# bhargav0410/gpu-accel-ofdm-ls-mrc

Measured on AMD Instinct MI355X. Metric: OFDM symbols/s (LS+MRC) at 1024 subcarriers x 64 ant; achieved HBM GB/s vs peak, higher is better.
Workload: dtype f32; 1 GPU; OFDM uplink LS+MRC, time-domain IQ in HBM, 1250 frames x 101 symbols (1 pilot + 100 data) x 64 antennas x 1024 subcarriers per GPU; domain=time, R=64, C=1024, S=101, prefix=0, frames_per_gpu=1250, data_symbols_per_gpu=125000, global_data_symbols=125000, flow=one-launch, parallelism=frame-sharded x1, no collective

## Files before the change

### gpu-accel-ofdm-ls-mrc_amd/csrc/frame_td.hip

```cpp
#include "launch.hpp"
#include "wave_fft1024.hpp"
#include "diag.hpp"

OFDM_DIAG_TU(td1024)


namespace ofdm {
namespace td1024 {

constexpr int LS_WAVES = 4;

template <int NW, class IQ>
__global__ void __launch_bounds__(64 * NW) k_ls_td1024(const IQ *__restrict__ iq, int S, int R,
                                                       int prefix, const float2 *__restrict__ X,
                                                       float2 *__restrict__ Hc, float *__restrict__ P,
                                                       int partial, float scale) {
    extern __shared__ __attribute__((aligned(16))) float2 lds[];
    float2 *tw = lds;
    const int w = threadIdx.x >> 6;
    const int t = threadIdx.x & 63;
    float2 *T = lds + TWBUF + w * TBUF;
    fill_twiddles(tw);
    __syncthreads();

    const long long f = blockIdx.x;
    const int Cp = C + prefix;
    const IQ *pilot = iq + f * (long long)S * R * Cp + prefix;
    float4 *Hf = reinterpret_cast<float4 *>(Hc + f * (long long)R * C);
    const int b0 = lane_bin0(t);
    float2 xp[16];
#pragma unroll
    for (int k = 0; k < 16; ++k) {
        const int b = b0 + 16 * k;
        xp[k] = b > 0 ? X[b - 1] : float2{1.f, 0.f};
    }
    float p[16];
#pragma unroll
    for (int k = 0; k < 16; ++k) p[k] = 0.f;
    for (int r = w; r < R; r += NW) {
        float2 a[16], x[16];
        if constexpr (is_sc16<IQ>) {
            unsigned raw[16];
            row_load(pilot + (long long)r * Cp, t, raw);
            widen_row(raw, a);
        } else {
            row_load(pilot + (long long)r * Cp, t, a);
        }
        row_fft(a, t, T, tw, x);
#pragma unroll
        for (int k = 0; k < 16; ++k) {
            float2 h = ls_conj(x[k], xp[k]);
            if constexpr (is_sc16<IQ>) h = float2{h.x * scale, h.y * scale};
            if (b0 + 16 * k == 0) h = float2{0.f, 0.f};
            x[k] = h;
            p[k] = p[k] + (h.x * h.x) + (h.y * h.y);
        }
        hc_store(Hf + (long long)r * (C / 2), t, x);
    }
    __syncthreads();
    float *pp = reinterpret_cast<float *>(lds + TWBUF);
    static_assert(NW * C * sizeof(float) <= NW * TBUF * sizeof(float2), "partials fit the transpose images");
#pragma unroll
    for (int k = 0; k < 16; ++k) pp[w * C + b0 + 16 * k] = p[k];
    __syncthreads();
    float *Pf = P + f * C;
    const int nw = R < NW ? R : NW;
    for (int b = threadIdx.x; b < C; b += blockDim.x) {
        float sum = pp[b];
        for (int i = 1; i < nw; ++i) sum = sum + pp[i * C + b];
        Pf[b] = b == 0 ? (partial ? 0.f : 1.f) : sum;
    }
}


__device__ __forceinline__ void fft_a(float2 (&a)[16], int t, float2 *T, const float2 *tw1) {
    hlds::row_fft_a<0, false, true>(a, t, T, tw1);
}
__device__ __forceinline__ void fft_b(int t, float2 *T, const float2 *tw2, float2 (&x)[16]) {
    hlds::row_fft_b<0, false, true>(t, T, tw2, x);
}
__device__ __forceinline__ void mac(float2 &acc, float2 x, float vx, float vy) {
    acc.x = __builtin_fmaf(-x.y, vy, __builtin_fmaf(x.x, vx, acc.x));
    acc.y = __builtin_fmaf(x.y, vx, __builtin_fmaf(x.x, vy, acc.y));
}


typedef int v4i_t __attribute__((ext_vector_type(4)));
template <bool PREF, class IQ>
__device__ __forceinline__ void hlds_row_pf(const IQ *next, __amdgpu_buffer_rsrc_t hc, int hoff, int t,
                                            row_reg_t<IQ> (&a)[16],
                                            float2 *T, const float2 *tw1, const float2 *tw2,
                                            const float4 *lo, const float4 *hi, float4 *mine,
                                            float2 (&acc)[16]) {
    using namespace hlds;
    float2 x[16];
    if constexpr (is_sc16<IQ>) {
        float2 af[16];
        widen_row(a, af);
        fft_a(af, t, T, tw1);
    } else {
        fft_a(a, t, T, tw1);
    }
    const float4 hreg = __builtin_bit_cast(float4, (v4i_t)__builtin_amdgcn_raw_buffer_load_b128(hc, t * 16, hoff, 0));
    __builtin_amdgcn_sched_barrier(0);
    if (PREF) row_load<true>(next, t, a);
    fft_b(t, T, tw2, x);
    if constexpr (is_sc16<IQ>) __builtin_amdgcn_sched_barrier(0);
    lds_barrier();
    *mine = hreg;
    lds_barrier();
#pragma unroll
    for (int i = 0; i < 8; ++i) {
        const float4 v = i < 4 ? lo[i * 64] : hi[(i - 4) * TS];
        mac(acc[2 * i], x[2 * i], v.x, v.y);
        mac(acc[2 * i + 1], x[2 * i + 1], v.z, v.w);
    }
}

template <bool R0, class IQ>
__device__ __forceinline__ void row0(const IQ *sym, int t, const float2 *T, row_reg_t<IQ> (&a)[16]) {
    if constexpr (R0) {
        static_assert(!is_sc16<IQ>, "sc16 rows are only 4-byte aligned: no 16-B row-0 DMA");
        asm volatile("s_waitcnt vmcnt(0)" ::: "memory");
#pragma unroll
        for (int m = 0; m < 16; ++m) a[m] = T[t + 64 * m];
    } else {
        row_load<true>(sym, t, a);
    }
}
__device__ __forceinline__ void row0_dma(const float2 *sym, int t, float2 *T) {
    const char *src = reinterpret_cast<const char *>(sym) + t * 16;
    const unsigned dst = lds_addr(T);
#pragma unroll
    for (int j = 0; j < 8; ++j) dma16(src + j * 1024, dst + j * 1024);
}

template <bool SHARED, bool R0 = false, class IQ>
__device__ __forceinline__ void hlds_rows(const IQ *sym, int Cp, int R, const float4 *Hf, int t,
                                          float2 *T, const float2 *tw1, const float2 *tw2,
                                          float2 *T0, float4 *hfree, float2 (&acc)[16]) {
    using namespace hlds;
#pragma unroll
    for (int k = 0; k < 16; ++k) acc[k] = float2{0.f, 0.f};
    if constexpr (SHARED) {
        row_reg_t<IQ> a[16];
        const int tl = lane_here();
        row0<R0>(sym, tl, T, a);
        const float4 *lo = hfree + tl;
        const float4 *hi = hslot(T0, hfree, 256 + tl);
        float4 *mine = hslot(T0, hfree, threadIdx.x);
        const __amdgpu_buffer_rsrc_t hc =
            __builtin_amdgcn_make_buffer_rsrc(const_cast<float4 *>(Hf), (short)0, R * (C * 8), 0x00020000);
        const int hw = __builtin_amdgcn_readfirstlane(threadIdx.x >> 6) * 1024;
        for (int r = 0; r + 1 < R; ++r)
            hlds_row_pf<true>(sym + (long long)(r + 1) * Cp, hc, r * (C * 8) + hw, lane_here(), a, T, tw1, tw2, lo,
                              hi, mine, acc);
        hlds_row_pf<false>(sym, hc, (R - 1) * (C * 8) + hw, lane_here(), a, T, tw1, tw2, lo, hi, mine, acc);
    } else {
        for (int r = 0; r < R; ++r) {
            float2 a[16], x[16], h[16];
            if constexpr (is_sc16<IQ>) {
                unsigned raw[16];
                if (r == 0)
                    row0<R0>(sym, t, T, raw);
                else
                    row_load<true>(sym + (long long)r * Cp, t, raw);
                widen_row(raw, a);
            } else if (r == 0) {
                row0<R0>(sym, t, T, a);
            } else {
                row_load<true>(sym + (long long)r * Cp, t, a);
            }
            fft_a(a, t, T, tw1);
            fft_b(t, T, tw2, x);
            __builtin_amdgcn_sched_barrier(0);
            hc_load(Hf + (long long)r * (C / 2), t, h);
#pragma unroll
            for (int k = 0; k < 16; ++k) mac(acc[k], x[k], h[k].x, h[k].y);
        }
    }
}

template <bool SCALED = false>
__device__ __forceinline__ void hlds_epilogue(const float2 (&acc)[16], const float *P, long long f, long long q,
                                              int t, float2 *T, float2 *__restrict__ out, int mode,
                                              float scale = 1.f) {
    const int b0 = lane_bin0(t);
    float2 *o = out + q * K;
    const float *Pf = P + f * C + b0;
    float pv[16];
    if ((mode & 1) == 0) {
#pragma unroll
        for (int k = 0; k < 16; ++k) pv[k] = Pf[16 * k];
    }
#pragma unroll
    for (int k = 0; k < 16; ++k) {
        const int b = b0 + 16 * k;
        float2 v = acc[k];
        int j = b - 1;
        if ((mode & 1) == 0) {
            float rp = __builtin_amdgcn_rcpf(pv[k]);
            if constexpr (SCALED) rp = rp * scale;
            v = float2{acc[k].x * rp, acc[k].y * rp};
            j = out_pos(b > 0 ? b - 1 : 0, K);
        } else if constexpr (SCALED) {
            v = float2{acc[k].x * scale, acc[k].y * scale};
        }
        if (b > 0) T[(j >> 6) * hlds::TP + (j & 63)] = v;
    }
    wave_lds_sync();
#pragma unroll
    for (int m = 0; m < 16; ++m) {
        const int j = t + 64 * m;
        if (j < K) {
            const float2 v = T[m * hlds::TP + t];
            __builtin_nontemporal_store(__builtin_bit_cast(unsigned long long, v),
                                        reinterpret_cast<unsigned long long *>(o + j));
        }
    }
}

template <bool R0, class IQ>
__global__ void __attribute__((amdgpu_flat_work_group_size(512, 512), amdgpu_waves_per_eu(4, 4)))
k_mrc_td1024_hlds(const IQ *__restrict__ iq, int S, int R, int prefix, const float2 *__restrict__ Hc,
                  const float *__restrict__ P, float2 *__restrict__ out, long long nq, long long nblocks,
                  long long per_xcd, int mode, float scale) {
    using namespace hlds;
    constexpr int HW = WAVES;
    extern __shared__ __attribute__((aligned(16))) float2 lds[];
    float2 *tw1 = lds, *tw2 = lds + TW1S;
    const int w = __builtin_amdgcn_readfirstlane(threadIdx.x >> 6), t = threadIdx.x & 63;
    float2 *T = lds + TW1S + TW2S + w * TS;
    float2 *T0 = lds + TW1S + TW2S;
    float4 *hfree = reinterpret_cast<float4 *>(T0 + HW * TS);
    const long long pb = blockIdx.x;
    const long long lb = (pb & 7) * per_xcd + (pb >> 3);
    if (lb >= nblocks) return;

    const int nsym = S - 1;
    const long long qw = lb * HW + w;
    const bool store = qw < nq;
    const long long q = store ? qw : nq - 1;
    const long long f = uniform64(q / nsym);
    const long long f0 = (lb * HW) / nsym;
    const long long fl = ((lb * HW + HW - 1 < nq ? lb * HW + HW - 1 : nq - 1)) / nsym;
    const int s = 1 + (int)(q % nsym);
    const int Cp = C + prefix;
    const IQ *sym = iq + (f * S + s) * (long long)R * Cp + prefix;
    if constexpr (R0) row0_dma(sym, t, T);
    fill(tw1, tw2);
    __syncthreads();

    float2 acc[16];
    if (f0 == fl)
        hlds_rows<true, R0>(sym, Cp, R, reinterpret_cast<const float4 *>(Hc + f0 * (long long)R * C), t, T,
                                 tw1, tw2, T0, hfree, acc);
    else
        hlds_rows<false, R0>(sym, Cp, R, reinterpret_cast<const float4 *>(Hc + f * (long long)R * C), t, T,
                                tw1, tw2, T0, hfree, acc);
    if (!store) return;
    if constexpr (is_sc16<IQ>)
        hlds_epilogue<true>(acc, P, f, q, lane_here(), T, out, mode, scale);
    else
        hlds_epilogue(acc, P, f, q, lane_here(), T, out, mode);
}


__device__ __forceinline__ void hlds_ls_frame(const float2 *__restrict__ iq, int S, int R, int prefix,
                                              const float2 *__restrict__ X, float2 *Hc, float *P, long long f,
                                              int w, int t, float2 *T, float2 *T0, const float2 *tw1,
                                              const float2 *tw2, unsigned long long *mx = nullptr) {
    using namespace hlds;
    (void)mx;
    const int Cp = C + prefix;
    const float2 *pilot = iq + f * (long long)S * R * Cp + prefix;
    float4 *Hf = reinterpret_cast<float4 *>(Hc + f * (long long)R * C);
    const int b0 = lane_bin0(t);
    float2 xp[16];
#pragma unroll
    for (int k = 0; k < 16; ++k) {
        const int b = b0 + 16 * k;
        xp[k] = b > 0 ? X[b - 1] : float2{1.f, 0.f};
    }
    float p[16];
#pragma unroll
    for (int k = 0; k < 16; ++k) p[k] = 0.f;
    for (int r = w; r < R; r += WAVES) {
        float2 a[16], x[16];
        const int tl = lane_here();
        row_load<true>(pilot + (long long)r * Cp, tl, a);
        fft_a(a, tl, T, tw1);
        fft_b(tl, T, tw2, x);
#pragma unroll
        for (int k = 0; k < 16; ++k) {
            float2 h = ls_conj(x[k], xp[k]);
            if (b0 + 16 * k == 0) h = float2{0.f, 0.f};
            x[k] = h;
            p[k] = p[k] + (h.x * h.x) + (h.y * h.y);
        }
#pragma unroll
        for (int i = 0; i < 8; ++i) store16_wt(Hf, R * C * 8, (r * (C / 2) + i * 64 + tl) * 16, x[2 * i], x[2 * i + 1]);
        if (r == w) {
            OFDM_DIAG_MARKP(mx, 1)
        }
    }
    OFDM_DIAG_MARKP(mx, 2)
    __syncthreads();
    float *pp = reinterpret_cast<float *>(T0);
#pragma unroll
    for (int k = 0; k < 16; ++k) pp[w * C + b0 + 16 * k] = p[k];
    __syncthreads();
    float *Pf = P + f * C;
    const int nw = R < WAVES ? R : WAVES;
    for (int b = threadIdx.x; b < C; b += blockDim.x) {
        float sum = pp[b];
        for (int i = 1; i < nw; ++i) sum = sum + pp[i * C + b];
        const float v = b == 0 ? 1.f : sum;
        store4_wt(Pf + b, v);
    }
    OFDM_DIAG_MARKP(mx, 3)
    __syncthreads();
}

__device__ __forceinline__ void split_unit(const float2 *__restrict__ iq, int S, int R, int prefix, const float2 *Hc,
                                           const float *P, float2 *__restrict__ out, long long nq, long long q0, int w,
                                           int t, float2 *T, float2 *T0, const float2 *tw1, const float2 *tw2) {
    const int nsym = S - 1, Cp = C + prefix, hh = w >> 2, R0 = (R + 1) >> 1;
    const long long qw = q0 + (w & 3);
    const bool store = qw < nq;
    const long long q = store ? qw : nq - 1;
    const long long f = q / nsym;
    const int s = 1 + (int)(q % nsym);
    const float2 *sym = iq + (f * S + s) * (long long)R * Cp + prefix;
    const float4 *Hf = reinterpret_cast<const float4 *>(Hc + f * (long long)R * C);
    float2 acc[16];
#pragma unroll
    for (int k = 0; k < 16; ++k) acc[k] = float2{0.f, 0.f};
    const int r1 = hh ? R : R0;
    for (int r = hh ? R0 : 0; r < r1; ++r) {
        float2 a[16], x[16], h[16];
        row_load<true>(sym + (long long)r * Cp, t, a);
        fft_a(a, t, T, tw1);
        fft_b(t, T, tw2, x);
        __builtin_amdgcn_sched_barrier(0);
        hc_load(Hf + (long long)r * (C / 2), t, h);
#pragma unroll
        for (int k = 0; k < 16; ++k) mac(acc[k], x[k], h[k].x, h[k].y);
    }
    if (hh) {
#pragma unroll
        for (int k = 0; k < 16; ++k) T[k * hlds::TP + t] = acc[k];
    }
    __syncthreads();
    if (hh) return;
    const float2 *Tp = T0 + (w + 4) * hlds::TS;
#pragma unroll
    for (int k = 0; k < 16; ++k) {
        const float2 v = Tp[k * hlds::TP + t];
        acc[k] = float2{acc[k].x + v.x, acc[k].y + v.y};
    }
    if (store) hlds_epilogue(acc, P, f, q, t, T, out, 0);
}

__global__ void __attribute__((amdgpu_flat_work_group_size(512, 512), amdgpu_waves_per_eu(4, 4)))
k_demod_td1024(const float2 *__restrict__ iq, int S, int R, int prefix, const float2 *__restrict__ X, float2 *Hc,
               float *P, float2 *__restrict__ out, long long nq, long long nblocks, Tickets tk, long long k0, long long split, unsigned long long *flags, unsigned long long epoch,
               int nls, long long nframes, long long spin_ticks) {
    using namespace hlds;
    constexpr int HW = WAVES;
    extern __shared__ __attribute__((aligned(16))) float2 lds[];
    float2 *tw1 = lds, *tw2 = lds + TW1S;
    const int w = __builtin_amdgcn_readfirstlane(threadIdx.x >> 6), t = threadIdx.x & 63;
    float2 *T = lds + TW1S + TW2S + w * TS;
    float2 *T0 = lds + TW1S + TW2S;
    float4 *hfree = reinterpret_cast<float4 *>(T0 + HW * TS);
    OFDM_DIAG_BEGIN()

    const bool estimator = (int)blockIdx.x < nls;
    auto first_frame = [&](long long lb) { return (lb * HW) / (S - 1); };
    auto last_frame = [&](long long lb) { return ((lb * HW + HW - 1 < nq ? lb * HW + HW - 1 : nq - 1)) / (S - 1); };
    const int nsym = S - 1, Cp = C + prefix;
    auto sym_of = [&](long long lb) {
        const long long qw = lb * HW + w, q = qw < nq ? qw : nq - 1;
        return iq + ((q / nsym) * S + 1 + q % nsym) * (long long)R * Cp + prefix;
    };
    long long e0 = 1, e1 = 0, lb = 0;
    int um = 0;
    if (estimator) {
        e0 = e1 = blockIdx.x;
        if (e0 >= nframes) return;
        __builtin_amdgcn_s_setprio(3);
        fill(tw1, tw2);
        __syncthreads();
        OFDM_DIAG_MARKN(0)
    } else {
        FillRegs fr;
        fill_load(fr);
        lb = wg_take_unit(tk, nblocks, k0, (long long)blockIdx.x - nls, split,
                          reinterpret_cast<long long *>(hfree + 255));
        if (lb < 0) return;
        OFDM_DIAG_MARKN(0)
        um = (int)(lb & 3);
        lb >>= 2;
        fill_store(tw1, tw2, fr);
        const long long f0 = first_frame(lb), fl = last_frame(lb);
        if (!um) row0_dma(sym_of(lb), t, T);
        bool seen_before = false;
        if (threadIdx.x == 0)
            seen_before = __hip_atomic_load((gu64 *)(flags + f0), __ATOMIC_RELAXED, __HIP_MEMORY_SCOPE_AGENT) == epoch &&
                          __hip_atomic_load((gu64 *)(flags + fl), __ATOMIC_RELAXED, __HIP_MEMORY_SCOPE_AGENT) == epoch;
        OFDM_DIAG_MARKN(1)
        if (!consume_flags(flags, f0, fl, epoch, spin_ticks, reinterpret_cast<int *>(hfree), seen_before)) {
            asm volatile("s_waitcnt vmcnt(0)" ::: "memory");
            __syncthreads();
            e0 = f0;
            e1 = fl;
        }
    }
    for (long long ff = e0; ff <= e1; ++ff)
        hlds_ls_frame(iq, S, R, prefix, X, Hc, P, ff, w, t, T, T0, tw1, tw2, OFDM_DIAG_ARG);
    if (estimator) {
        OFDM_DIAG_MARK()
        publish_flag(flags + e0, epoch, w == 0 && lane_here() == 0);
        OFDM_DIAG_END_SLOT(td1024, epoch);
        return;
    }
    if (e0 <= e1) {
        acquire_all();
        if (!um) row0_dma(sym_of(lb), t, T);
    }
    OFDM_DIAG_MARK()

    if (um) {
        split_unit(iq, S, R, prefix, Hc, P, out, nq, lb * HW + 4 * (um - 1), w, t, T, T0, tw1, tw2);
        OFDM_DIAG_END_SLOT(td1024, epoch);
        return;
    }
    const long long qw = lb * HW + w;
    const bool store = qw < nq;
    const long long q = store ? qw : nq - 1;
    const long long f = q / nsym;
    const long long f0 = first_frame(lb), fl = last_frame(lb);
    const float2 *sym = sym_of(lb);
    float2 acc[16];
    if (f0 == fl)
        hlds_rows<true, true>(sym, Cp, R, reinterpret_cast<const float4 *>(Hc + f0 * (long long)R * C), t, T,
                              tw1, tw2, T0, hfree, acc);
    else
        hlds_rows<false, true>(sym, Cp, R, reinterpret_cast<const float4 *>(Hc + f * (long long)R * C), t, T,
                               tw1, tw2, T0, hfree, acc);
    OFDM_DIAG_MARKN(2)
    if (store) hlds_epilogue(acc, P, f, q, lane_here(), T, out, 0);
    OFDM_DIAG_END_SLOT(td1024, epoch);
}

}

namespace {
template <class IQ>
hipError_t ls_td1024(const IQ *iq, long long nframes, int S, int R, int prefix, float scale,
                     const float2 *X, float2 *Hc, float *P, int partial, hipStream_t s) {
    using namespace td1024;
    if (nframes <= 0) return hipSuccess;
    if (nframes > 0x7fffffffll) return hipErrorInvalidValue;
    int nw = (nframes * LS_WAVES < 2048 && R > LS_WAVES) ? 16 : LS_WAVES;
    auto k16 = k_ls_td1024<16, IQ>;
    auto k4 = k_ls_td1024<LS_WAVES, IQ>;
    auto k8 = k16;
    if (nw == 16 || nw == 8) {
        auto kern = nw == 16 ? k16 : k8;
        const size_t lds = (TWBUF + nw * TBUF) * sizeof(float2);
        if (hipError_t e = opt_in_lds(reinterpret_cast<const void *>(kern), (int)lds); e != hipSuccess) return e;
        hipLaunchKernelGGL(kern, dim3((unsigned)nframes), dim3(64 * nw), lds, s, iq, S, R, prefix, X, Hc, P,
                           partial, scale);
        return hipGetLastError();
    }
    const size_t lds = (TWBUF + LS_WAVES * TBUF) * sizeof(float2);
    hipLaunchKernelGGL(k4, dim3((unsigned)nframes), dim3(64 * LS_WAVES), lds, s, iq, S, R, prefix, X, Hc, P,
                       partial, scale);
    return hipGetLastError();
}

template <class IQ>
hipError_t mrc_td1024(const IQ *iq, long long nframes, int S, int R, int prefix, float scale,
                      const float2 *Hc, const float *P, float2 *out, int mode, hipStream_t s) {
    using namespace td1024;
    const long long nq = nframes * (S - 1);
    if (nq <= 0) return hipSuccess;
    const long long nb = (nq + hlds::WAVES - 1) / hlds::WAVES;
    const long long pxcd = (nb + 7) / 8;
    if (pxcd * 8 > 0x7fffffffll) return hipErrorInvalidValue;
    auto kern = k_mrc_td1024_hlds<!is_sc16<IQ>, IQ>;
    hipLaunchKernelGGL(kern, dim3((unsigned)(pxcd * 8)), dim3(64 * hlds::WAVES), hlds::LDS_BYTES, s, iq, S, R,
                       prefix, Hc, P, out, nq, nb, pxcd, mode, scale);
    return hipGetLastError();
}
}

hipError_t launch_ls_td1024(const float2 *iq, long long nframes, int S, int R, int prefix,
                            const float2 *X, float2 *Hc, float *P, int partial, hipStream_t s) {
    return ls_td1024(iq, nframes, S, R, prefix, 1.f, X, Hc, P, partial, s);
}
hipError_t launch_ls_td1024_sc16(const sc16 *iq, long long nframes, int S, int R, int prefix, float scale,
                                 const float2 *X, float2 *Hc, float *P, int partial, hipStream_t s) {
    return ls_td1024(iq, nframes, S, R, prefix, scale, X, Hc, P, partial, s);
}
hipError_t launch_mrc_td1024(const float2 *iq, long long nframes, int S, int R, int prefix,
                             const float2 *Hc, const float *P, float2 *out, int mode,
                             hipStream_t s) {
    return mrc_td1024(iq, nframes, S, R, prefix, 1.f, Hc, P, out, mode, s);
}
hipError_t launch_mrc_td1024_sc16(const sc16 *iq, long long nframes, int S, int R, int prefix, float scale,
                                  const float2 *Hc, const float *P, float2 *out, int mode, hipStream_t s) {
    return mrc_td1024(iq, nframes, S, R, prefix, scale, Hc, P, out, mode, s);
}

hipError_t launch_demod_td1024(const float2 *iq, long long nframes, int S, int R, int prefix, const float2 *X,
                               float2 *Hc, float *P, float2 *out, Tickets tk,
                               unsigned long long *flags, unsigned long long epoch, long long spin_ticks,
                               hipStream_t s) {
    using namespace td1024;
    const long long nq = nframes * (S - 1);
    if (nq <= 0) return hipSuccess;
    const long long nb = (nq + hlds::WAVES - 1) / hlds::WAVES;
    const long long nls = (nframes + 7) / 8 * 8;
    const long long k1 = ticket_k0(2), k0 = 2 * k1, split = R >= 2 ? k1 : 0;
    const long long g = ticket_grid(nb, 8 * split);
    if (g + nls > 0x7fffffffll) return hipErrorInvalidValue;
    hipLaunchKernelGGL(k_demod_td1024, dim3((unsigned)(nls + g)), dim3(64 * hlds::WAVES), hlds::LDS_BYTES, s, iq,
                       S, R, prefix, X, Hc, P, out, nq, nb, tk, k0, split, flags, epoch, (int)nls, nframes,
                       spin_ticks < 0 ? SPIN_TICKS : spin_ticks);
    return hipGetLastError();
}

}
```

### gpu-accel-ofdm-ls-mrc_amd/csrc/wave_fft1024.hpp

```cpp
#pragma once
#include "common.hpp"
#include "launch.hpp"
#include "pk.hpp"

namespace ofdm {
namespace td1024 {

constexpr int C = 1024;
constexpr int K = C - 1;
constexpr int TP = 68;
constexpr int TBUF = 16 * TP;
constexpr int TW1P = 17;
constexpr int TW1BUF = 64 * TW1P;
constexpr int TW2P = 17;
constexpr int TW2BUF = 4 * TW2P;
constexpr int TWBUF = TW1BUF + TW2BUF;

__device__ __forceinline__ void wave_lds_sync() {
    __builtin_amdgcn_fence(__ATOMIC_RELEASE, "wavefront");
    __builtin_amdgcn_wave_barrier();
    __builtin_amdgcn_fence(__ATOMIC_ACQUIRE, "wavefront");
}

__device__ __forceinline__ void lds_barrier() {
    asm volatile("s_waitcnt lgkmcnt(0)\n\ts_barrier" ::: "memory");
}

typedef __attribute__((address_space(3))) void lvoid_t;
__device__ __forceinline__ unsigned lds_addr(const void *p) { return (unsigned)(size_t)(lvoid_t *)p; }

__device__ __forceinline__ void dma16(const void *g, unsigned lds) {
    unsigned keep;
    asm volatile("s_mov_b32 %0, m0\n\ts_mov_b32 m0, %2\n\ts_nop 0\n\tglobal_load_lds_dwordx4 %1, off\n\t"
                 "s_mov_b32 m0, %0"
                 : "=&s"(keep)
                 : "v"(g), "s"(lds)
                 : "memory");
}

__device__ __forceinline__ float quad_g(int a) { return (a == 0 || a == 3) ? 1.f : -1.f; }

__device__ __forceinline__ void fill_twiddles(float2 *tw) {
    for (int i = threadIdx.x; i < TW1BUF; i += blockDim.x) {
        const int t = i / TW1P, k2 = i % TW1P;
        tw[i] = k2 < 16 ? g_tw[((t * k2) & (C - 1)) * (OFDM_TW_N / C)] : float2{0.f, 0.f};
    }
    for (int i = threadIdx.x; i < TW2BUF; i += blockDim.x) {
        const int a = i / TW2P, k = i % TW2P;
        const float2 w = g_tw[((16 * a * k) & (C - 1)) * (OFDM_TW_N / C)];
        const float g = quad_g(a);
        tw[TW1BUF + i] = k < 16 ? float2{g * w.x, g * w.y} : float2{0.f, 0.f};
    }
}

template <int CTRL>
__device__ __forceinline__ float dpp(float v) {
    return __builtin_bit_cast(float, __builtin_amdgcn_mov_dpp(__builtin_bit_cast(int, v), CTRL,
                                                              0xF, 0xF, true));
}
constexpr int DPP_XOR1 = 0xB1;
constexpr int DPP_XOR2 = 0x4E;

template <bool NT = false>
__device__ __forceinline__ void row_load(const float2 *__restrict__ src, int t, float2 (&a)[16]) {
    if (NT) {
        const unsigned long long *p = reinterpret_cast<const unsigned long long *>(src) + t;
#pragma unroll
        for (int m = 0; m < 16; ++m)
            a[m] = __builtin_bit_cast(float2, __builtin_nontemporal_load(p + 64 * m));
    } else {
#pragma unroll
        for (int m = 0; m < 16; ++m) a[m] = src[t + 64 * m];
    }
}

template <class IQ>
struct row_regs {
    typedef float2 type;
};
template <>
struct row_regs<sc16> {
    typedef unsigned type;
};
template <class IQ>
using row_reg_t = typename row_regs<IQ>::type;
template <class IQ>
constexpr bool is_sc16 = __is_same(IQ, sc16);

template <bool NT = false>
__device__ __forceinline__ void row_load(const sc16 *__restrict__ src, int t, unsigned (&a)[16]) {
    const unsigned *p = reinterpret_cast<const unsigned *>(src) + t;
#pragma unroll
    for (int m = 0; m < 16; ++m) a[m] = NT ? __builtin_nontemporal_load(p + 64 * m) : p[64 * m];
}
__device__ __forceinline__ float2 widen(unsigned v) {
    return float2{(float)(short)(v & 0xffffu), (float)((int)v >> 16)};
}
__device__ __forceinline__ void widen_row(const unsigned (&a)[16], float2 (&x)[16]) {
#pragma unroll
    for (int m = 0; m < 16; ++m) x[m] = widen(a[m]);
}

#define OFDM_DPP_Q(CTRL) "quad_perm:" CTRL " row_mask:0xf bank_mask:0xf"
template <int CTRL>
__device__ __forceinline__ void quad_fmac_dpp(float (&v)[16], float S) {
#define OFDM_F(i) "v_fmac_f32_dpp %" #i ", %" #i ", %16 " OFDM_DPP_Q(QP) "\n\t"
    if constexpr (CTRL == 0x4E) {
#define QP "[2,3,0,1]"
        asm("s_nop 1\n\t" OFDM_F(0) OFDM_F(1) OFDM_F(2) OFDM_F(3) OFDM_F(4) OFDM_F(5) OFDM_F(6)
                OFDM_F(7) OFDM_F(8) OFDM_F(9) OFDM_F(10) OFDM_F(11) OFDM_F(12) OFDM_F(13) OFDM_F(14)
                    OFDM_F(15)
            : "+v"(v[0]), "+v"(v[1]), "+v"(v[2]), "+v"(v[3]), "+v"(v[4]), "+v"(v[5]), "+v"(v[6]),
              "+v"(v[7]), "+v"(v[8]), "+v"(v[9]), "+v"(v[10]), "+v"(v[11]), "+v"(v[12]),
              "+v"(v[13]), "+v"(v[14]), "+v"(v[15])
            : "v"(S));
#undef QP
    } else {
        static_assert(CTRL == 0xB1, "quad xor 1 or xor 2");
#define QP "[1,0,3,2]"
        asm("s_nop 1\n\t" OFDM_F(0) OFDM_F(1) OFDM_F(2) OFDM_F(3) OFDM_F(4) OFDM_F(5) OFDM_F(6)
                OFDM_F(7) OFDM_F(8) OFDM_F(9) OFDM_F(10) OFDM_F(11) OFDM_F(12) OFDM_F(13) OFDM_F(14)
                    OFDM_F(15)
            : "+v"(v[0]), "+v"(v[1]), "+v"(v[2]), "+v"(v[3]), "+v"(v[4]), "+v"(v[5]), "+v"(v[6]),
              "+v"(v[7]), "+v"(v[8]), "+v"(v[9]), "+v"(v[10]), "+v"(v[11]), "+v"(v[12]),
              "+v"(v[13]), "+v"(v[14]), "+v"(v[15])
            : "v"(S));
#undef QP
    }
#undef OFDM_F
}
#undef OFDM_DPP_Q

__device__ __forceinline__ void quad_dft(float2 (&x)[16], int qa) {
    const float S1 = (qa & 2) ? 1.f : -1.f;
    const float S2 = (qa & 1) ? 1.f : -1.f;
    const unsigned long long rot = __builtin_amdgcn_ballot_w64(qa == 3);
    float xr[16], xi[16];
#pragma unroll
    for (int k = 0; k < 16; ++k) { xr[k] = x[k].x; xi[k] = x[k].y; }
    quad_fmac_dpp<DPP_XOR2>(xr, S1);
    quad_fmac_dpp<DPP_XOR2>(xi, S1);
#pragma unroll
    for (int k = 0; k < 16; ++k) {
        float nx;
        asm("v_cndmask_b32_e64 %0, %2, %3, %4\n\tv_cndmask_b32_e64 %1, %3, -%2, %4"
            : "=&v"(nx), "=v"(xi[k])
            : "v"(xr[k]), "v"(xi[k]), "s"(rot));
        xr[k] = nx;
    }
    quad_fmac_dpp<DPP_XOR1>(xr, S2);
    quad_fmac_dpp<DPP_XOR1>(xi, S2);
#pragma unroll
    for (int k = 0; k < 16; ++k) x[k] = float2{xr[k], xi[k]};
}

__device__ __forceinline__ void row_fft(float2 (&a)[16], int t, float2 *T, const float2 *tw,
                                        float2 (&x)[16]) {
    fft16_fma(a);
#pragma unroll
    for (int k2 = 1; k2 < 16; ++k2) a[k2] = cmul(a[k2], tw[t * TW1P + k2]);
#pragma unroll
    for (int k2 = 0; k2 < 16; ++k2) T[k2 * TP + t] = a[k2];
    wave_lds_sync();
    const int q = t >> 2, qa = t & 3;
#pragma unroll
    for (int l = 0; l < 16; ++l) x[l] = T[q * TP + qa + 4 * l];
    wave_lds_sync();
    fft16_fma(x);
    const float2 *tw2 = tw + TW1BUF + qa * TW2P;
    const float g = quad_g(qa);
    x[0] = float2{g * x[0].x, g * x[0].y};
#pragma unroll
    for (int k = 1; k < 16; ++k) x[k] = cmul(x[k], tw2[k]);
    quad_dft(x, qa);
}

__device__ __forceinline__ int lane_bin0(int t) {
    const int qa = t & 3;
    return (t >> 2) + 256 * ((qa >> 1) + 2 * (qa & 1));
}

__device__ __forceinline__ int nat_img(int n) { return (n >> 6) * TP + (((n & 63) + 4 * (n >> 8)) & 63); }

__device__ __forceinline__ void hc_store(float4 *__restrict__ dst, int t, const float2 (&h)[16]) {
#pragma unroll
    for (int i = 0; i < 8; ++i)
        dst[i * 64 + t] = float4{h[2 * i].x, h[2 * i].y, h[2 * i + 1].x, h[2 * i + 1].y};
}
__device__ __forceinline__ void hc_load(const float4 *__restrict__ src, int t, float2 (&h)[16]) {
#pragma unroll
    for (int i = 0; i < 8; ++i) {
        const float4 v = src[i * 64 + t];
        h[2 * i] = float2{v.x, v.y};
        h[2 * i + 1] = float2{v.z, v.w};
    }
}

typedef __attribute__((address_space(1))) unsigned long long gu64;
typedef __attribute__((address_space(1))) unsigned gu32;
constexpr long long SPIN_TICKS = 200000;

__device__ __forceinline__ void store16_wt(const void *base, int bytes, int off, float2 a, float2 b) {
    typedef int v4i __attribute__((ext_vector_type(4)));
    const __amdgpu_buffer_rsrc_t rs =
        __builtin_amdgcn_make_buffer_rsrc(const_cast<void *>(base), (short)0, bytes, 0x00020000);
    const v4i v = {__builtin_bit_cast(int, a.x), __builtin_bit_cast(int, a.y), __builtin_bit_cast(int, b.x),
                   __builtin_bit_cast(int, b.y)};
    __builtin_amdgcn_raw_buffer_store_b128(v, rs, off, 0, 16);
}
__device__ __forceinline__ void store8_wt(float2 *p, float2 v) {
    __hip_atomic_store((gu64 *)(p), __builtin_bit_cast(unsigned long long, v), __ATOMIC_RELAXED,
                       __HIP_MEMORY_SCOPE_AGENT);
}
__device__ __forceinline__ void store4_wt(float *p, float v) {
    __hip_atomic_store((gu32 *)(p), __builtin_bit_cast(unsigned, v), __ATOMIC_RELAXED, __HIP_MEMORY_SCOPE_AGENT);
}

__device__ __forceinline__ void publish_flag(unsigned long long *flag, unsigned long long epoch, bool one) {
    asm volatile("s_waitcnt vmcnt(0)" ::: "memory");
    __syncthreads();
    if (one) {
        asm volatile("s_waitcnt vmcnt(0)" ::: "memory");
        __hip_atomic_store((gu64 *)(flag), epoch, __ATOMIC_RELAXED, __HIP_MEMORY_SCOPE_AGENT);
    }
}

__device__ __forceinline__ bool wait_flag(unsigned long long *flag, unsigned long long epoch, long long ticks) {
    const long long t0 = wall_clock64();
    while (__hip_atomic_load((gu64 *)(flag), __ATOMIC_RELAXED, __HIP_MEMORY_SCOPE_AGENT) != epoch) {
        if (wall_clock64() - t0 >= ticks) return false;
        __builtin_amdgcn_s_sleep(2);
    }
    return true;
}

__device__ __forceinline__ bool consume_flags(unsigned long long *flags, long long f0, long long fl,
                                              unsigned long long epoch, long long ticks, int *seen,
                                              bool seen_before = false) {
    if (threadIdx.x == 0) {
        bool ok = true;
        if (!seen_before)
            for (long long f = f0; f <= fl && ok; ++f) ok = wait_flag(flags + f, epoch, ticks);
        *seen = ok ? 1 : 0;
        if (ok) __builtin_amdgcn_fence(__ATOMIC_ACQUIRE, "agent");
        asm volatile("s_waitcnt vmcnt(0)" ::: "memory");
    }
    __syncthreads();
    const bool ok = *seen != 0;
    __syncthreads();
    return ok;
}
__device__ __forceinline__ void acquire_all() {
    asm volatile("s_waitcnt vmcnt(0)" ::: "memory");
    __syncthreads();
    if (threadIdx.x == 0) {
        __builtin_amdgcn_fence(__ATOMIC_ACQUIRE, "agent");
        asm volatile("s_waitcnt vmcnt(0)" ::: "memory");
    }
    __syncthreads();
}

constexpr int TICKET_STRIDE = 16;
constexpr int HWREG_XCC_ID = (31 << 11) | 20;
__device__ __forceinline__ long long ticket_range_count(long long nb, long long per, unsigned y) {
    const long long lo = (long long)y * per;
    return nb - lo < per ? (nb - lo > 0 ? nb - lo : 0) : per;
}
__device__ __forceinline__ void ticket_fault(const Tickets &tk, unsigned why) {
    if (tk.status) __hip_atomic_store((gu32 *)tk.status, why, __ATOMIC_RELAXED, __HIP_MEMORY_SCOPE_SYSTEM);
}
__device__ __forceinline__ long long take_ticket(const Tickets &tk, unsigned y, long long units) {
    gu64 *p = (gu64 *)(tk.set + y * TICKET_STRIDE);
    const unsigned long long mine = (unsigned long long)tk.tag << 32;
    unsigned long long v = __hip_atomic_load(p, __ATOMIC_RELAXED, __HIP_MEMORY_SCOPE_AGENT);
    for (int tries = 0; (v >> 32) != tk.tag; ++tries) {
        if (tries == 64) {
            ticket_fault(tk, TK_CONTENDED);
            return -2;
        }
        if (__hip_atomic_compare_exchange_strong(p, &v, mine | 1ull, __ATOMIC_RELAXED, __ATOMIC_RELAXED,
                                                 __HIP_MEMORY_SCOPE_AGENT))
            return 0;
    }
    if ((long long)(unsigned)v >= units) return -1;
    const unsigned long long r = __hip_atomic_fetch_add(p, 1ull, __ATOMIC_RELAXED, __HIP_MEMORY_SCOPE_AGENT);
    if ((r >> 32) != tk.tag) {
        ticket_fault(tk, TK_FOREIGN);
        return -2;
    }
    const long long t = (long long)(unsigned)r;
    if (t < units) return t;
    if (t > units + (long long)gridDim.x) ticket_fault(tk, TK_RANGE);
    return -1;
}
__device__ __forceinline__ long long uniform64(long long v) {
    const int lo = __builtin_amdgcn_readfirstlane((int)(v & 0xffffffffll));
    const int hi = __builtin_amdgcn_readfirstlane((int)(v >> 32));
    return (long long)(((unsigned long long)(unsigned)hi << 32) | (unsigned)lo);
}
__device__ __forceinline__ long long take_unit(const Tickets &tk, long long nb, long long k0, long long pb,
                                               long long split) {
    const long long per = (nb + 7) / 8;
    if (pb < 8 * k0) {
        const unsigned y = (unsigned)(pb & 7);
        const long long k = pb >> 3, cnt = ticket_range_count(nb, per, y);
        if (k < (cnt < k0 ? cnt : k0)) return ((long long)y * per + k) << 2;
    }
    const unsigned x = (unsigned)__builtin_amdgcn_s_getreg(HWREG_XCC_ID) & 7u;
    for (int j = 0; j < 8; ++j) {
        const unsigned y = (x + (unsigned)j) & 7u;
        const long long cnt = ticket_range_count(nb, per, y), s0 = cnt < k0 ? cnt : k0;
        const long long avail = cnt - s0;
        if (avail <= 0) continue;
        const long long ns = split < avail ? split : avail, whole = avail - ns;
        const long long t = take_ticket(tk, y, whole + 2 * ns);
        if (t < 0) continue;
        const long long b0 = (long long)y * per + s0;
        if (t < whole) return (b0 + t) << 2;
        const long long u = t - whole;
        return ((b0 + whole + (u >> 1)) << 2) | (1 + (u & 1));
    }
    return -1;
}
__device__ __forceinline__ long long wg_take_unit(const Tickets &tk, long long nb, long long k0, long long pb,
                                                  long long split, long long *slot) {
    if (threadIdx.x == 0) {
        if (pb == 0) {
#pragma unroll
            for (int y = 0; y < 8; ++y)
                __hip_atomic_store((gu64 *)(tk.set + y * TICKET_STRIDE), (unsigned long long)tk.tag << 32,
                                   __ATOMIC_RELAXED, __HIP_MEMORY_SCOPE_AGENT);
        }
        *slot = take_unit(tk, nb, k0, pb, split);
    }
    __syncthreads();
    const long long v = *slot;
    return uniform64(v);
}
__device__ __forceinline__ long long wg_take_block(const Tickets &tk, long long nb, long long k0, long long pb,
                                                   long long *slot) {
    const long long u = wg_take_unit(tk, nb, k0, pb, 0, slot);
    return u < 0 ? u : u >> 2;
}
inline long long ticket_grid(long long nb, long long split_units = 0) { return nb + split_units + nb / 4 + 64; }
inline long long ticket_k0(int per_cu) {
    static const int cus = [] {
        int dev = 0, n = 256;
        if (hipGetDevice(&dev) != hipSuccess || hipDeviceGetAttribute(&n, hipDeviceAttributeMultiprocessorCount, dev) != hipSuccess)
            n = 256;
        return n;
    }();
    return (long long)per_cu * cus / 8;
}

namespace hlds {
constexpr int TW1S = 15 * 64;
constexpr int TW2S = 16 * 4;
constexpr int TP = 68;
constexpr int TS = 16 * TP;
constexpr int WAVES = 8;
constexpr size_t LDS_BYTES = (TW1S + TW2S + WAVES * TS) * sizeof(float2) + 256 * sizeof(float4);
static_assert(LDS_BYTES == 81920, "two workgroups per CU");

__device__ __forceinline__ float4 *hslot(float2 *T0, float4 *hfree, int j) {
    if (j < 256) return hfree + j;
    const int jj = j - 256;
    return reinterpret_cast<float4 *>(T0 + (jj >> 5) * TS + ((jj >> 1) & 15) * TP + 64 + 2 * (jj & 1));
}

__device__ __forceinline__ void fill(float2 *tw1, float2 *tw2) {
    for (int i = threadIdx.x; i < TW1S; i += blockDim.x) {
        const int k2 = 1 + i / 64, t = i % 64;
        tw1[i] = g_tw[((t * k2) & (C - 1)) * (OFDM_TW_N / C)];
    }
    for (int i = threadIdx.x; i < TW2S; i += blockDim.x) {
        const int k = i / 4, a = i % 4;
        const float2 w = g_tw[((16 * a * k) & (C - 1)) * (OFDM_TW_N / C)];
        const float g = quad_g(a);
        tw2[i] = float2{g * w.x, g * w.y};
    }
}
struct FillRegs {
    float2 v[3];
};
__device__ __forceinline__ void fill_load(FillRegs &f) {
    const int i0 = threadIdx.x, i1 = threadIdx.x + 512;
    auto w1 = [](int i) { return g_tw[(((i % 64) * (1 + i / 64)) & (C - 1)) * (OFDM_TW_N / C)]; };
    f.v[0] = w1(i0);
    f.v[1] = i1 < TW1S ? w1(i1) : float2{0.f, 0.f};
    f.v[2] = i0 < TW2S ? g_tw[((16 * (i0 % 4) * (i0 / 4)) & (C - 1)) * (OFDM_TW_N / C)] : float2{0.f, 0.f};
}
__device__ __forceinline__ void fill_store(float2 *tw1, float2 *tw2, const FillRegs &f) {
    const int i0 = threadIdx.x, i1 = threadIdx.x + 512;
    tw1[i0] = f.v[0];
    if (i1 < TW1S) tw1[i1] = f.v[1];
    if (i0 < TW2S) {
        const float g = quad_g(i0 % 4);
        tw2[i0] = float2{g * f.v[2].x, g * f.v[2].y};
    }
}
static_assert(TW1S <= 1024 && TW2S <= 512, "fill_load covers the tables with 512 threads");
__device__ __forceinline__ int swz(int row, int col) { return row * TP + col; }

template <int N>
__device__ __forceinline__ void tw_powers(pk::v2f (&v)[N], pk::v2f w, pk::v2f sw) {
    const pk::v2f w2 = pk::cmul(w, w);
    pk::v2f po = sw, pe = pk::cmul(sw, w);
    v[1] = pk::cmul(v[1], po);
    v[2] = pk::cmul(v[2], pe);
#pragma unroll
    for (int k = 3; k < N; k += 2) {
        po = pk::cmul(po, w2);
        v[k] = pk::cmul(v[k], po);
        if (k + 1 < N) {
            pe = pk::cmul(pe, w2);
            v[k + 1] = pk::cmul(v[k + 1], pe);
        }
    }
}

template <int PK = 0, bool TWR = false, bool FMA = false>
__device__ __forceinline__ void row_fft_a(float2 (&a)[16], int t, float2 *T, const float2 *tw1) {
    if constexpr (TWR) {
        pk::v2f v[16];
#pragma unroll
        for (int m = 0; m < 16; ++m) v[m] = pk::V(a[m]);
        if constexpr ((PK & 1) != 0) {
            pk::fft_reg<16>(v);
        } else {
#pragma unroll
            for (int m = 0; m < 16; ++m) a[m] = pk::F(v[m]);
            fft_reg<16, false>(a);
#pragma unroll
            for (int m = 0; m < 16; ++m) v[m] = pk::V(a[m]);
        }
        const pk::v2f w = pk::V(tw1[t]);
        tw_powers(v, w, w);
#pragma unroll
        for (int k2 = 0; k2 < 16; ++k2) T[swz(k2, t)] = pk::F(v[k2]);
        return;
    }
    if constexpr (PK & 1) {
        pk::v2f v[16];
#pragma unroll
        for (int m = 0; m < 16; ++m) v[m] = pk::V(a[m]);
        pk::fft_reg<16>(v);
#pragma unroll
        for (int k2 = 1; k2 < 16; ++k2) v[k2] = pk::cmul(v[k2], pk::V(tw1[(k2 - 1) * 64 + t]));
#pragma unroll
        for (int k2 = 0; k2 < 16; ++k2) T[swz(k2, t)] = pk::F(v[k2]);
        return;
    }
    static_assert(!FMA || (PK == 0 && !TWR), "fft16_fma is the plain-f32 table-twiddle path's");
    if constexpr (FMA)
        fft16_fma(a);
    else
        fft_reg<16, false>(a);
#pragma unroll
    for (int k2 = 1; k2 < 16; ++k2) a[k2] = cmul(a[k2], tw1[(k2 - 1) * 64 + t]);
#pragma unroll
    for (int k2 = 0; k2 < 16; ++k2) T[swz(k2, t)] = a[k2];
}
template <int PK = 0, bool TWR = false, bool FMA = false>
__device__ __forceinline__ void row_fft_b(int t, float2 *T, const float2 *tw2, float2 (&x)[16]) {
    wave_lds_sync();
    const int q = t >> 2, qa = t & 3;
#pragma unroll
    for (int l = 0; l < 16; ++l) x[l] = T[swz(q, qa + 4 * l)];
    wave_lds_sync();
    const float g = quad_g(qa);
    if constexpr (TWR) {
        pk::v2f v[16];
        if constexpr ((PK & 2) != 0) {
#pragma unroll
            for (int m = 0; m < 16; ++m) v[m] = pk::V(x[m]);
            pk::fft_reg<16>(v);
        } else {
            fft_reg<16, false>(x);
#pragma unroll
            for (int m = 0; m < 16; ++m) v[m] = pk::V(x[m]);
        }
        v[0] = pk::scale(v[0], g);
        const pk::v2f gw = pk::V(tw2[4 + qa]);
        tw_powers(v, pk::scale(gw, g), gw);
#pragma unroll
        for (int m = 0; m < 16; ++m) x[m] = pk::F(v[m]);
    } else if constexpr (PK & 2) {
        pk::v2f v[16];
#pragma unroll
        for (int m = 0; m < 16; ++m) v[m] = pk::V(x[m]);
        pk::fft_reg<16>(v);
        v[0] = pk::scale(v[0], g);
#pragma unroll
        for (int k = 1; k < 16; ++k) v[k] = pk::cmul(v[k], pk::V(tw2[k * 4 + qa]));
#pragma unroll
        for (int m = 0; m < 16; ++m) x[m] = pk::F(v[m]);
    } else {
        static_assert(!FMA || (PK == 0 && !TWR), "fft16_fma is the plain-f32 table-twiddle path's");
        if constexpr (FMA)
            fft16_fma(x);
        else
            fft_reg<16, false>(x);
        x[0] = float2{g * x[0].x, g * x[0].y};
#pragma unroll
        for (int k = 1; k < 16; ++k) x[k] = cmul(x[k], tw2[k * 4 + qa]);
    }
    quad_dft(x, qa);
}
constexpr int TP16 = 72;
constexpr int TS16 = 16 * TP16;
__device__ __forceinline__ int perm16(int c) { return 8 * (c >> 3) + 2 * (c & 3) + ((c >> 2) & 1); }
__device__ __forceinline__ void fa_write16(const pk::v2f (&v)[16], int pt, float2 *T) {
#pragma unroll
    for (int k2 = 0; k2 < 16; ++k2) T[k2 * TP16 + pt] = pk::F(v[k2]);
}
__device__ __forceinline__ void fb_read16(int t, const float2 *T, pk::v2f (&v)[16]) {
    const float4 *s = reinterpret_cast<const float4 *>(T + (t >> 2) * TP16 + 2 * (t & 3));
#pragma unroll
    for (int j = 0; j < 8; ++j) {
        const float4 x = s[4 * j];
        v[2 * j] = pk::V(float2{x.x, x.y});
        v[2 * j + 1] = pk::V(float2{x.z, x.w});
    }
}

struct TwAnchors {
    pk::v2f w, a1, a4, a8, a12;
};
__device__ __forceinline__ void tw_anchored(pk::v2f (&v)[16], const TwAnchors &c) {
    const pk::v2f w2 = pk::cmul(c.w, c.w), w3 = pk::cmul(w2, c.w);
    v[1] = pk::cmul(v[1], c.a1);
    v[2] = pk::cmul(v[2], pk::cmul(c.a1, c.w));
    v[3] = pk::cmul(v[3], pk::cmul(c.a1, w2));
#pragma unroll
    for (int j = 1; j < 4; ++j) {
        const pk::v2f a = j == 1 ? c.a4 : j == 2 ? c.a8 : c.a12;
        v[4 * j] = pk::cmul(v[4 * j], a);
        v[4 * j + 1] = pk::cmul(v[4 * j + 1], pk::cmul(a, c.w));
        v[4 * j + 2] = pk::cmul(v[4 * j + 2], pk::cmul(a, w2));
        v[4 * j + 3] = pk::cmul(v[4 * j + 3], pk::cmul(a, w3));
    }
}
__device__ __forceinline__ TwAnchors anchors_a(const float2 *tw1, int t) {
    const pk::v2f w = pk::V(tw1[t]);
    return TwAnchors{w, w, pk::V(tw1[3 * 64 + t]), pk::V(tw1[7 * 64 + t]), pk::V(tw1[11 * 64 + t])};
}
__device__ __forceinline__ TwAnchors anchors_b(const float2 *tw2, int t) {
    const int qa = t & 3;
    const pk::v2f gw = pk::V(tw2[4 + qa]);
    return TwAnchors{pk::scale(gw, quad_g(qa)), gw, pk::V(tw2[16 + qa]), pk::V(tw2[32 + qa]), pk::V(tw2[48 + qa])};
}

__device__ __forceinline__ void fa_compute(pk::v2f (&v)[16], pk::v2f w1) {
    pk::fft_reg<16>(v);
    tw_powers(v, w1, w1);
}
__device__ __forceinline__ void fa_compute(pk::v2f (&v)[16], const TwAnchors &c) {
    pk::fft_reg<16>(v);
    tw_anchored(v, c);
}
__device__ __forceinline__ void fa_write(const pk::v2f (&v)[16], int t, float2 *T) {
#pragma unroll
    for (int k2 = 0; k2 < 16; ++k2) T[swz(k2, t)] = pk::F(v[k2]);
}
__device__ __forceinline__ void fb_read(int t, const float2 *T, pk::v2f (&v)[16]) {
    const int q = t >> 2, qa = t & 3;
#pragma unroll
    for (int l = 0; l < 16; ++l) v[l] = pk::V(T[swz(q, qa + 4 * l)]);
}
__device__ __forceinline__ void fb_compute(pk::v2f (&v)[16], pk::v2f gw, int t, float2 (&x)[16]) {
    const int qa = t & 3;
    const float g = quad_g(qa);
    pk::fft_reg<16>(v);
    v[0] = pk::scale(v[0], g);
    tw_powers(v, pk::scale(gw, g), gw);
#pragma unroll
    for (int m = 0; m < 16; ++m) x[m] = pk::F(v[m]);
    quad_dft(x, qa);
}
__device__ __forceinline__ void fb_compute(pk::v2f (&v)[16], const TwAnchors &c, int t, float2 (&x)[16]) {
    const int qa = t & 3;
    pk::fft_reg<16>(v);
    v[0] = pk::scale(v[0], quad_g(qa));
    tw_anchored(v, c);
#pragma unroll
    for (int m = 0; m < 16; ++m) x[m] = pk::F(v[m]);
    quad_dft(x, qa);
}

}

}
}
```

Measured before the change: 10.65 million symbols/s.

## Double-buffer row registers and spread next-row prefetch across FFT stages

For float2 input in the shared-H path, the per-antenna row loop now ping-pongs between two register arrays. The next row's 16 nontemporal loads are split into chunks issued between fft_a, fft_b, the LDS barriers and the MAC, instead of being issued in one block. The goal is to overlap HBM loads with FFT compute more evenly and avoid a single burst of outstanding loads. The cost is a second 16-entry row buffer per lane, which raises register pressure and may hurt occupancy. The row-0 wait also changes from an inline-asm vmcnt(0) to the builtin s_waitcnt.

```diff
diff --git a/gpu-accel-ofdm-ls-mrc_amd/csrc/frame_td.hip b/gpu-accel-ofdm-ls-mrc_amd/csrc/frame_td.hip
--- a/gpu-accel-ofdm-ls-mrc_amd/csrc/frame_td.hip
+++ b/gpu-accel-ofdm-ls-mrc_amd/csrc/frame_td.hip
@@ -117,11 +117,54 @@
     }
 }
 
+constexpr int PP_A = 4, PP_B = 8, PP_C = 4;
+template <bool PREF, class IQ>
+__device__ __forceinline__ void hlds_row_pp(const IQ *next, __amdgpu_buffer_rsrc_t hc, int hoff, int t,
+                                            row_reg_t<IQ> (&cur)[16], row_reg_t<IQ> (&nxt)[16],
+                                            float2 *T, const float2 *tw1, const float2 *tw2,
+                                            const float4 *lo, const float4 *hi, float4 *mine,
+                                            float2 (&acc)[16]) {
+    using namespace hlds;
+    static_assert(PP_A >= 0 && PP_B >= 0 && PP_C >= 0 && PP_A + PP_B + PP_C <= 16, "the row's 16 loads");
+    const float4 hreg = __builtin_bit_cast(float4, (v4i_t)__builtin_amdgcn_raw_buffer_load_b128(hc, t * 16, hoff, 0));
+    if (PREF) row_load_part<0, PP_A>(next, t, nxt);
+    __builtin_amdgcn_sched_barrier(0);
+    auto rest = [&](float2 (&x)[16]) {
+        fft_a(x, t, T, tw1);
+        __builtin_amdgcn_sched_barrier(0);
+        if (PREF) row_load_part<PP_A, PP_A + PP_B>(next, t, nxt);
+        __builtin_amdgcn_sched_barrier(0);
+        fft_b(t, T, tw2, x);
+        __builtin_amdgcn_sched_barrier(0);
+        if (PREF) row_load_part<PP_A + PP_B, PP_A + PP_B + PP_C>(next, t, nxt);
+        __builtin_amdgcn_sched_barrier(0);
+        lds_barrier();
+        *mine = hreg;
+        lds_barrier();
+        if (PREF) row_load_part<PP_A + PP_B + PP_C, 16>(next, t, nxt);
+        __builtin_amdgcn_sched_barrier(0);
+#pragma unroll
+        for (int i = 0; i < 8; ++i) {
+            const float4 v = i < 4 ? lo[i * 64] : hi[(i - 4) * TS];
+            mac(acc[2 * i], x[2 * i], v.x, v.y);
+            mac(acc[2 * i + 1], x[2 * i + 1], v.z, v.w);
+        }
+    };
+    if constexpr (is_sc16<IQ>) {
+        float2 x[16];
+        widen_row(cur, x);
+        rest(x);
+    } else {
+        rest(cur);
+    }
+}
+
 template <bool R0, class IQ>
 __device__ __forceinline__ void row0(const IQ *sym, int t, const float2 *T, row_reg_t<IQ> (&a)[16]) {
     if constexpr (R0) {
         static_assert(!is_sc16<IQ>, "sc16 rows are only 4-byte aligned: no 16-B row-0 DMA");
-        asm volatile("s_waitcnt vmcnt(0)" ::: "memory");
+        __builtin_amdgcn_s_waitcnt(0x0F70);
+        asm volatile("" ::: "memory");
 #pragma unroll
         for (int m = 0; m < 16; ++m) a[m] = T[t + 64 * m];
     } else {
@@ -145,17 +188,38 @@
     if constexpr (SHARED) {
         row_reg_t<IQ> a[16];
         const int tl = lane_here();
-        row0<R0>(sym, tl, T, a);
         const float4 *lo = hfree + tl;
         const float4 *hi = hslot(T0, hfree, 256 + tl);
         float4 *mine = hslot(T0, hfree, threadIdx.x);
         const __amdgpu_buffer_rsrc_t hc =
             __builtin_amdgcn_make_buffer_rsrc(const_cast<float4 *>(Hf), (short)0, R * (C * 8), 0x00020000);
         const int hw = __builtin_amdgcn_readfirstlane(threadIdx.x >> 6) * 1024;
-        for (int r = 0; r + 1 < R; ++r)
-            hlds_row_pf<true>(sym + (long long)(r + 1) * Cp, hc, r * (C * 8) + hw, lane_here(), a, T, tw1, tw2, lo,
-                              hi, mine, acc);
-        hlds_row_pf<false>(sym, hc, (R - 1) * (C * 8) + hw, lane_here(), a, T, tw1, tw2, lo, hi, mine, acc);
+        if constexpr (is_sc16<IQ>) {
+            row0<R0>(sym, tl, T, a);
+            for (int r = 0; r + 1 < R; ++r)
+                hlds_row_pf<true>(sym + (long long)(r + 1) * Cp, hc, r * (C * 8) + hw, lane_here(), a, T, tw1, tw2,
+                                  lo, hi, mine, acc);
+            hlds_row_pf<false>(sym, hc, (R - 1) * (C * 8) + hw, lane_here(), a, T, tw1, tw2, lo, hi, mine, acc);
+        } else {
+            row_reg_t<IQ> b[16];
+            auto row = [&](auto pref, int r, row_reg_t<IQ>(&cur)[16], row_reg_t<IQ>(&nxt)[16]) {
+                hlds_row_pp<decltype(pref)::value>(sym + (long long)(r + 1) * Cp, hc, r * (C * 8) + hw, lane_here(), cur,
+                                                   nxt, T, tw1, tw2, lo, hi, mine, acc);
+            };
+            int r = 0;
+            if ((R & 1) == 0) {
+                row0<R0>(sym, tl, T, b);
+                row(std::true_type{}, 0, b, a);
+                r = 1;
+            } else {
+                row0<R0>(sym, tl, T, a);
+            }
+            for (; r + 2 < R; r += 2) {
+                row(std::true_type{}, r, a, b);
+                row(std::true_type{}, r + 1, b, a);
+            }
+            row(std::false_type{}, r, a, b);
+        }
     } else {
         for (int r = 0; r < R; ++r) {
             float2 a[16], x[16], h[16];
diff --git a/gpu-accel-ofdm-ls-mrc_amd/csrc/wave_fft1024.hpp b/gpu-accel-ofdm-ls-mrc_amd/csrc/wave_fft1024.hpp
--- a/gpu-accel-ofdm-ls-mrc_amd/csrc/wave_fft1024.hpp
+++ b/gpu-accel-ofdm-ls-mrc_amd/csrc/wave_fft1024.hpp
@@ -92,6 +92,18 @@
     const unsigned *p = reinterpret_cast<const unsigned *>(src) + t;
 #pragma unroll
     for (int m = 0; m < 16; ++m) a[m] = NT ? __builtin_nontemporal_load(p + 64 * m) : p[64 * m];
+}
+template <int M0, int M1>
+__device__ __forceinline__ void row_load_part(const float2 *__restrict__ src, int t, float2 (&a)[16]) {
+    const unsigned long long *p = reinterpret_cast<const unsigned long long *>(src) + t;
+#pragma unroll
+    for (int m = M0; m < M1; ++m) a[m] = __builtin_bit_cast(float2, __builtin_nontemporal_load(p + 64 * m));
+}
+template <int M0, int M1>
+__device__ __forceinline__ void row_load_part(const sc16 *__restrict__ src, int t, unsigned (&a)[16]) {
+    const unsigned *p = reinterpret_cast<const unsigned *>(src) + t;
+#pragma unroll
+    for (int m = M0; m < M1; ++m) a[m] = __builtin_nontemporal_load(p + 64 * m);
 }
 __device__ __forceinline__ float2 widen(unsigned v) {
     return float2{(float)(short)(v & 0xffffu), (float)((int)v >> 16)};
```

Result: faster. 10.92 million symbols/s (median of 6 runs) (+2.5%).
